# rezashkv/diffusion_pruning

Hardware: AMD Instinct MI355X
Metric: denoise-steps/s (SD-2.1 U-Net forward, 512x512, bs=4 per GPU, 50% channel mask) (higher is better)
Workload: dtype bf16; 1 GPU; BASELINE configs[1]: SD-2.1 UNet2DConditionModelGated.forward, 64x64 latents (512x512), bs=4/GPU, fixed 50% mask (gated semantics), seeded random-init weights, HIP graph replay; global_batch=4, parallelism=replicas x1 (no data-path collective)

## Files before the change

diffusion_pruning_amd/csrc/conv_gemm.hip:

```cpp
#include "conv_gemm_core.h"

using namespace aptp_cg;

namespace {

template <typename T> struct Elem;
template <> struct Elem<__bf16> { static constexpr int EPC = 8, KS = 64; };
template <> struct Elem<float> { static constexpr int EPC = 4, KS = 32; };

template <int BM, int BN, int WM, int WN, typename T = __bf16>
__global__ __launch_bounds__(256) void conv_gemm_kernel(const KParams p) {
  static_assert(WM * WN == 4, "4 waves per workgroup");
  constexpr int EPC = Elem<T>::EPC, KS = Elem<T>::KS, ES = (int)sizeof(T);
  constexpr bool F32 = sizeof(T) == 4;
  constexpr int WTM = BM / WM, WTN = BN / WN;
  constexpr int MF = WTM / 16, NF = WTN / 16;
  constexpr int A_PASS = BM / 32, B_PASS = BN / 32;
  static_assert(BM % 32 == 0 && BN % 32 == 0 && WTM % 16 == 0 && WTN % 16 == 0, "tile shape");

  __shared__ __attribute__((aligned(16))) T smem[2 * (BM + BN) * KS];
  T* As = smem;
  T* Bs = smem + 2 * BM * KS;

  const int tid = threadIdx.x, lane = tid & 63, wave = tid >> 6;
// ... 1016 lines not shown
void launch_tile(const KParams& k, hipStream_t s) {
  const int tiles = ((k.M + BM - 1) / BM) * ((k.N + BN - 1) / BN);
  dim3 grid(tiles * k.split_k, 1, 1);
  if (k.io_f32) hipLaunchKernelGGL((conv_gemm_kernel<BM, BN, 2, 2, float>), grid, dim3(256), 0, s, k);
  else hipLaunchKernelGGL((conv_gemm_kernel<BM, BN, 2, 2>), grid, dim3(256), 0, s, k);
}

template <int BM, int BN, int STAGES>
void launch_tile_dma(const KParams& k, hipStream_t s) {
  const int tiles = ((k.M + BM - 1) / BM) * ((k.N + BN - 1) / BN);
  dim3 grid(tiles * k.split_k, 1, 1);
  hipLaunchKernelGGL((conv_gemm_dma_kernel<BM, BN, 2, 2, STAGES>), grid, dim3(256), 0, s, k);
}

template <int BM, int BN, int WM, int WN, int STAGES = 2>
void launch_tile_dma8(const KParams& k, hipStream_t s) {
  const int tiles = ((k.M + BM - 1) / BM) * ((k.N + BN - 1) / BN);
  dim3 grid(tiles * k.split_k, 1, 1);
  hipLaunchKernelGGL((conv_gemm_dma_kernel<BM, BN, WM, WN, STAGES>), grid, dim3(512), 0, s, k);
}

template <int BM, int BN, int WM, int WN, int STAGES>
void launch_tile_ku2(const KParams& k, hipStream_t s) {
  const int tiles = ((k.M + BM - 1) / BM) * ((k.N + BN - 1) / BN);
  dim3 grid(tiles * k.split_k, 1, 1);
  hipLaunchKernelGGL((conv_gemm_dma_kernel<BM, BN, WM, WN, STAGES, false, 2>), grid, dim3(WM * WN * 64), 0, s, k);
}

template <int BM, int BN, int STAGES>
void launch_tile_ks2(const KParams& k, hipStream_t s) {
  const int tiles = ((k.M + BM - 1) / BM) * ((k.N + BN - 1) / BN);
  dim3 grid(tiles * k.split_k, 1, 1);
  hipLaunchKernelGGL((conv_gemm_dma_kernel<BM, BN, 2, 2, STAGES, false, 1, 2>), grid, dim3(512), 0, s, k);
}

template <int BM, int BN, int WM, int WN, int STAGES>
void launch_tile_pp(const KParams& k, hipStream_t s) {
  const int tiles = ((k.M + BM - 1) / BM) * ((k.N + BN - 1) / BN);
  dim3 grid(tiles * k.split_k, 1, 1);
  hipLaunchKernelGGL((conv_gemm_dma_kernel<BM, BN, WM, WN, STAGES, true>), grid, dim3(512), 0, s, k);
}

}

extern "C" int64_t aptp_conv_gemm_workspace_bytes(const AptpConvGemmParams* p) {
  if (!p || p->split_k <= 1) return 0;
  const int64_t M = (int64_t)p->B * p->Hout * p->Wout;
  const int t = pick_tile(p, (int)M);
  if (is_sk_tile(t))
    return (int64_t)aptp_sk_cus() * 2 * kTiles[t].bm * kTiles[t].bn * (int64_t)sizeof(float);
  int64_t mp = M, np = p->N;
  if (t > 0 && t < kNumTiles) {
    mp = (M + kTiles[t].bm - 1) / kTiles[t].bm * kTiles[t].bm;
    np = ((int64_t)p->N + kTiles[t].bn - 1) / kTiles[t].bn * kTiles[t].bn;
  }
  return (int64_t)p->split_k * mp * np * (int64_t)sizeof(float);
}

extern "C" int aptp_conv_gemm_tiles(const AptpConvGemmParams* p) {
  if (!p) return 0;
  const int64_t M = (int64_t)p->B * p->Hout * p->Wout;
  const int t = pick_tile(p, (int)M);
  if (t <= 0 || t >= kNumTiles) return 0;
  return (int)(((M + kTiles[t].bm - 1) / kTiles[t].bm) * ((p->N + kTiles[t].bn - 1) / kTiles[t].bn));
}

extern "C" int aptp_conv_gemm_colstat_rows(const AptpConvGemmParams* p) {
  if (!p) return 0;
  const int t = pick_tile(p, p->B * p->Hout * p->Wout);
  if (t <= 0 || t >= kNumTiles) return 0;
  return kTiles[t].bm / (kTiles[t].nw / kTiles[t].wn);
}

extern "C" int aptp_conv_gemm_rowstat_slots(const AptpConvGemmParams* p) {
  if (!p) return 0;
  const int t = pick_tile(p, p->B * p->Hout * p->Wout);
  if (t <= 0 || t >= kNumTiles) return 0;
  return ((p->N + kTiles[t].bn - 1) / kTiles[t].bn) * kTiles[t].wn;
}

extern "C" int aptp_conv_gemm_suggest_split_k(const AptpConvGemmParams* p) {
  if (!p) return 1;
  const int M = p->B * p->Hout * p->Wout;
  const int t = pick_tile(p, M);
  const int64_t blocks = (int64_t)((M + kTiles[t].bm - 1) / kTiles[t].bm) * ((p->N + kTiles[t].bn - 1) / kTiles[t].bn);
  const int nK = p->KH * p->KW * (p->cin_pad / BK);
  if (blocks >= 256) return 1;
  int s = (int)((512 + blocks - 1) / blocks);
  const int max_s = nK / 8 > 0 ? nK / 8 : 1;
  if (s > max_s) s = max_s;
  if (s > 32) s = 32;
  return s < 1 ? 1 : s;
}

extern "C" int aptp_conv_gemm(const AptpConvGemmParams* p, aptp_stream_t stream) {
  KParams k;
  const int rc = fill_kparams(p, k);
  if (rc != APTP_OK) return rc;
  if (k.split_k > 1) APTP_CHECK(k.ws != nullptr && ((uintptr_t)k.ws % 16) == 0, "conv_gemm: split_k > 1 needs a 16B-aligned workspace");
  if (k.split_k == 1) k.counters = nullptr;
  k.gn_gamma = p->gn_gamma; k.gn_beta = p->gn_beta; k.gn_groups = p->gn_groups; k.gn_C = p->gn_C; k.gn_silu = p->gn_silu; k.gn_eps = p->gn_eps;
  if (k.gn_gamma) {
    APTP_CHECK(k.gn_beta && k.split_k > 1 && !k.counters && !k.out_f32 && k.act == APTP_ACT_NONE && !k.colgate && !k.corr && !k.residual && !k.depth
               && !k.rstat_out && !k.cstat_out && !k.ln_stats, "conv_gemm: gn_gamma needs a plain bf16 convolution split along K with a reduce launch");
    APTP_CHECK(k.gn_groups > 0 && k.gn_C > 0 && k.gn_C <= k.N && k.gn_C % k.gn_groups == 0 && k.gn_C % 8 == 0 && (k.gn_C / k.gn_groups) % 4 == 0
               && (int64_t)k.HW * (k.gn_C / k.gn_groups) <= 4LL * GN_RED_QPT * GN_RED_NT && k.ldy % 4 == 0,
               "conv_gemm: gn_gamma geometry (C=%d groups=%d HW=%d)", k.gn_C, k.gn_groups, k.HW);
  }
  hipStream_t s = (hipStream_t)stream;
  int t = pick_tile(p, k.M);
  if (t < 0 || t >= kNumTiles) { aptp_set_error("conv_gemm: unknown tile %d", t); return APTP_EINVAL; }
  if (k.io_f32 && t >= APTP_TILE_DMA_128x128) {
    aptp_set_error("conv_gemm: io_f32 (fp32 parity path) runs on the register-staged tiles 1..6 only (got tile %d)", t);
    return APTP_EINVAL;
  }
  if (t >= APTP_TILE_DMA_128x128 && !is_sk_tile(t) && (p->cin_pad * 2 > 8064 || (p->x2 && p->cin2_pad * 2 > 8064))) {
    aptp_set_error("conv_gemm: LDS-DMA tiles need Cin <= 4032 (got cin_pad %d)", p->cin_pad);
    return APTP_EINVAL;
  }
  if (k.rstat_out) {
    const int slots = ((k.N + kTiles[t].bn - 1) / kTiles[t].bn) * kTiles[t].wn;
    if ((k.split_k != 1 && !k.counters) || k.rstat_slots != slots) {
      aptp_set_error("conv_gemm: rowstat_out needs split_k == 1 (or the in-kernel reduction) and rowstat_slots == aptp_conv_gemm_rowstat_slots() (%d), got split_k %d, slots %d",
                     slots, k.split_k, k.rstat_slots);
      return APTP_EINVAL;
    }
  }
  if (k.cstat_out) {
    const int wtm = kTiles[t].bm / (kTiles[t].nw / kTiles[t].wn), wtn = kTiles[t].bn / kTiles[t].wn;
    if (!k.epi16 || k.act == APTP_ACT_GEGLU || (k.split_k != 1 && !k.counters) || k.HW % wtm != 0 || wtn < 32 ||
        k.cstat_ld < k.Nout || ((uintptr_t)k.cstat_out % 8) != 0) {
      aptp_set_error("conv_gemm: colstat_out needs the coalesced bf16 epilogue, no GEGLU, split_k == 1 (or the in-kernel reduction), "
                     "Hout*Wout %% %d == 0 (aptp_conv_gemm_colstat_rows) and colstat_ld >= N", wtm);
      return APTP_EINVAL;
    }
    const int wl = k.act == APTP_ACT_GEGLU ? wtn / 2 : wtn;
    if (k.ustat_out && (wl % k.ustat_unit == 0 ? wl / k.ustat_unit : (wl - 1) / k.ustat_unit + 2) > 64) {
      aptp_set_error("conv_gemm: ustat_unit %d too small for the %d columns of a wave of tile %d (at most 64 units per wave)", k.ustat_unit, wl, t);
      return APTP_EINVAL;
    }
  }
  if (k.act == APTP_ACT_GEGLU && (kTiles[t].bn == 160)) {
    aptp_set_error("conv_gemm: GEGLU cannot use a 160-wide tile");
    return APTP_EINVAL;
  }
  {
    const int tiles_m = (k.M + kTiles[t].bm - 1) / kTiles[t].bm, tiles_n = (k.N + kTiles[t].bn - 1) / kTiles[t].bn;
    APTP_CHECK((int64_t)tiles_m * tiles_n * k.split_k < (1ll << 31) && (int64_t)k.nK * (k.split_k + 1) < (1ll << 31), "conv_gemm: grid too large");
    k.fd_hw = make_fastdiv(k.HW); k.fd_wout = make_fastdiv(k.Wout);
    k.fd_tm = make_fastdiv(tiles_m); k.fd_tn = make_fastdiv(tiles_n); k.fd_sk = make_fastdiv(k.split_k);
    k.fd_perm = make_fastdiv(tiles_n * k.split_k); k.fd_tmn = make_fastdiv(tiles_m * tiles_n);
  }
  static const bool lin_on = !(getenv("APTP_LIN") && getenv("APTP_LIN")[0] == '0');
  if (lin_on && p->epilogue != 2 && p->pad_end == 0 && aptp_lin_eligible(k, t)) {
    const int rc2 = aptp_launch_lin(k, t, s);
    if (rc2 != APTP_OK) return rc2;
    APTP_LAUNCH_CHECK();
    return APTP_OK;
  }
  static const bool lean_on = !(getenv("APTP_CONV_LEAN") && getenv("APTP_CONV_LEAN")[0] == '0');
  if (lean_on && p->epilogue == 0 && p->pad_end == 0 && aptp_conv_lean_eligible(k, t)) {
    const int rc2 = aptp_launch_conv_lean(k, t, s);
    if (rc2 != APTP_OK) return rc2;
  } else
  switch (t) {
    case APTP_TILE_128x128: launch_tile<128, 128>(k, s); break;
    case APTP_TILE_128x160: launch_tile<128, 160>(k, s); break;
    case APTP_TILE_64x128: launch_tile<64, 128>(k, s); break;
    case APTP_TILE_64x160: launch_tile<64, 160>(k, s); break;
    case APTP_TILE_128x64: launch_tile<128, 64>(k, s); break;
    case APTP_TILE_64x64: launch_tile<64, 64>(k, s); break;
    case APTP_TILE_DMA_128x128: launch_tile_dma<128, 128, 2>(k, s); break;
    case APTP_TILE_DMA_128x160: launch_tile_dma<128, 160, 2>(k, s); break;
    case APTP_TILE_DMA_64x128: launch_tile_dma<64, 128, 2>(k, s); break;
    case APTP_TILE_DMA_64x160: launch_tile_dma<64, 160, 2>(k, s); break;
    case APTP_TILE_DMA_128x64: launch_tile_dma<128, 64, 2>(k, s); break;
    case APTP_TILE_DMA_64x64: launch_tile_dma<64, 64, 2>(k, s); break;
    case APTP_TILE_DMA3_128x128: launch_tile_dma<128, 128, 3>(k, s); break;
    case APTP_TILE_DMA3_128x160: launch_tile_dma<128, 160, 3>(k, s); break;
    case APTP_TILE_DMA3_64x128: launch_tile_dma<64, 128, 3>(k, s); break;
    case APTP_TILE_DMA3_64x160: launch_tile_dma<64, 160, 3>(k, s); break;
    case APTP_TILE_DMA3_128x64: launch_tile_dma<128, 64, 3>(k, s); break;
    case APTP_TILE_DMA3_64x64: launch_tile_dma<64, 64, 3>(k, s); break;
    case APTP_TILE_DMA8_128x160: launch_tile_dma8<128, 160, 4, 2>(k, s); break;
    case APTP_TILE_DMA8_256x160: launch_tile_dma8<256, 160, 4, 2>(k, s); break;
    case APTP_TILE_DMA8_128x128: launch_tile_dma8<128, 128, 2, 4>(k, s); break;
    case APTP_TILE_DMA8_256x128: launch_tile_dma8<256, 128, 4, 2>(k, s); break;
    case APTP_TILE_DMA4_64x160: launch_tile_dma<64, 160, 4>(k, s); break;
    case APTP_TILE_DMA4_64x128: launch_tile_dma<64, 128, 4>(k, s); break;
    case APTP_TILE_DMA4_64x64: launch_tile_dma<64, 64, 4>(k, s); break;
    case APTP_TILE_DMA4_128x64: launch_tile_dma<128, 64, 4>(k, s); break;
    case APTP_TILE_DMA4_128x128: launch_tile_dma<128, 128, 4>(k, s); break;
    case APTP_TILE_DMA8R3_128x160: launch_tile_dma8<128, 160, 4, 2, 3>(k, s); break;
    case APTP_TILE_DMA8R4_128x160: launch_tile_dma8<128, 160, 4, 2, 4>(k, s); break;
    case APTP_TILE_DMA8R3_128x128: launch_tile_dma8<128, 128, 2, 4, 3>(k, s); break;
    case APTP_TILE_DMA8R4_128x128: launch_tile_dma8<128, 128, 2, 4, 4>(k, s); break;
    case APTP_TILE_DMA8R3_256x128: launch_tile_dma8<256, 128, 4, 2, 3>(k, s); break;
    case APTP_TILE_PP3_128x160: launch_tile_pp<128, 160, 4, 2, 3>(k, s); break;
    case APTP_TILE_PP4_128x160: launch_tile_pp<128, 160, 4, 2, 4>(k, s); break;
    case APTP_TILE_PP3_128x128: launch_tile_pp<128, 128, 2, 4, 3>(k, s); break;
    case APTP_TILE_PP4_128x128: launch_tile_pp<128, 128, 2, 4, 4>(k, s); break;
    case APTP_TILE_PP4_64x160: launch_tile_pp<64, 160, 4, 2, 4>(k, s); break;
    case APTP_TILE_PP4_64x128: launch_tile_pp<64, 128, 2, 4, 4>(k, s); break;
    case APTP_TILE_PP5_64x160: launch_tile_pp<64, 160, 4, 2, 5>(k, s); break;
    case APTP_TILE_PP4_128x64: launch_tile_pp<128, 64, 4, 2, 4>(k, s); break;
    case APTP_TILE_PP3_256x128: launch_tile_pp<256, 128, 4, 2, 3>(k, s); break;
    case APTP_TILE_PP3_128x256: launch_tile_pp<128, 256, 2, 4, 3>(k, s); break;
    case APTP_TILE_DMA6_64x64: launch_tile_dma<64, 64, 6>(k, s); break;
    case APTP_TILE_DMA8S_64x64: launch_tile_dma<64, 64, 8>(k, s); break;
    case APTP_TILE_DMA6_64x128: launch_tile_dma<64, 128, 6>(k, s); break;
    case APTP_TILE_DMA6_128x64: launch_tile_dma<128, 64, 6>(k, s); break;
    case APTP_TILE_KU2S4_64x64: launch_tile_ku2<64, 64, 2, 2, 4>(k, s); break;
    case APTP_TILE_KU2S6_64x64: launch_tile_ku2<64, 64, 2, 2, 6>(k, s); break;
    case APTP_TILE_KU2S4_64x128: launch_tile_ku2<64, 128, 2, 2, 4>(k, s); break;
    case APTP_TILE_KU2S6_64x128: launch_tile_ku2<64, 128, 2, 2, 6>(k, s); break;
    case APTP_TILE_KU2S4_128x64: launch_tile_ku2<128, 64, 2, 2, 4>(k, s); break;
    case APTP_TILE_KU2S4_128x128: launch_tile_ku2<128, 128, 2, 2, 4>(k, s); break;
    case APTP_TILE_KU2S4_64x160: launch_tile_ku2<64, 160, 2, 2, 4>(k, s); break;
    case APTP_TILE_KU2S4_128x160: launch_tile_ku2<128, 160, 4, 2, 4>(k, s); break;
    case APTP_TILE_KU2S4_128x128W8: launch_tile_ku2<128, 128, 2, 4, 4>(k, s); break;
    case APTP_TILE_KS2S3_64x64: launch_tile_ks2<64, 64, 3>(k, s); break;
    case APTP_TILE_KS2S4_64x64: launch_tile_ks2<64, 64, 4>(k, s); break;
    case APTP_TILE_KS2S3_64x128: launch_tile_ks2<64, 128, 3>(k, s); break;
    case APTP_TILE_KS2S4_64x128: launch_tile_ks2<64, 128, 4>(k, s); break;
    case APTP_TILE_KS2S3_128x64: launch_tile_ks2<128, 64, 3>(k, s); break;
    case APTP_TILE_KS2S3_128x128: launch_tile_ks2<128, 128, 3>(k, s); break;
    case APTP_TILE_SK_256x160: case APTP_TILE_SK_256x128: case APTP_TILE_SK_128x256:
    case APTP_TILE_SKL_256x160: case APTP_TILE_SKL_256x128: case APTP_TILE_SKL_128x256:
    case APTP_TILE_SK_128x160: case APTP_TILE_SKL_128x160: case APTP_TILE_SK_128x128: case APTP_TILE_SKL_128x128: {
      if (k.split_k > 1 && !k.counters) { aptp_set_error("conv_gemm: the stream-K tiles combine in-kernel: split_k > 1 needs tile_counters"); return APTP_EINVAL; }
      const int rc2 = aptp_launch_sk(k, t, s);
      if (rc2 != APTP_OK) return rc2;
      break;
    }
    case APTP_TILE_HALO_128x160:
    case APTP_TILE_HALO_128x128: {
      const int W = p->Wout;
      if (!(p->KH == 3 && p->KW == 3 && p->stride == 1 && p->pad == 1 && p->pad_end == 0 && p->ups == 0 && !p->x2 && W > 0 && 128 % W == 0 &&
            (p->Hout * W) % 128 == 0 && (128 / W + 2) * (W + 2) <= 264)) {
        aptp_set_error("conv_gemm: the halo tiles need a 3x3 / stride-1 / pad-1 convolution without x2 whose width divides 128 (16, 32 or 64)");
        return APTP_EINVAL;
      }
      const int tiles = ((k.M + 127) / 128) * ((k.N + kTiles[t].bn - 1) / kTiles[t].bn);
      if (t == APTP_TILE_HALO_128x160) hipLaunchKernelGGL((conv3x3_halo_kernel<160, 4>), dim3(tiles * k.split_k), dim3(512), 0, s, k);
      else hipLaunchKernelGGL((conv3x3_halo_kernel<128, 4>), dim3(tiles * k.split_k), dim3(512), 0, s, k);
      break;
    }
    default: aptp_set_error("conv_gemm: unknown tile %d", t); return APTP_EINVAL;
  }
  APTP_LAUNCH_CHECK();
  if (k.split_k > 1 && !k.counters) {
    if (k.gn_gamma) {
      hipLaunchKernelGGL(splitk_reduce_gn_kernel, dim3(k.gn_groups, k.B), dim3(GN_RED_NT), 0, s, k);
    } else {
      const int quads = (k.act == APTP_ACT_GEGLU) ? k.N / 8 : k.N / 4;
      const int64_t total = (int64_t)k.M * quads;
      hipLaunchKernelGGL(splitk_reduce_kernel, dim3((unsigned)((total + 255) / 256)), dim3(256), 0, s, k);
    }
    APTP_LAUNCH_CHECK();
  }
  return APTP_OK;
}
```

diffusion_pruning_amd/csrc/lin_gemm.hip:

```cpp
#include "conv_gemm_core.h"

namespace {
using namespace aptp_cg;

__device__ __attribute__((aligned(256))) unsigned char g_lin_zero_page[8192];

typedef __attribute__((address_space(3))) void* lds_ptr;
typedef const __attribute__((address_space(1))) void* gbl_ptr;

template <int BM, int BN, int WM, int WN, int STAGES, int KU, bool GEGLU = false, int GELU = 0>
__global__ __launch_bounds__(WM * WN * 64) void lin_gemm_kernel(const KParams p) {
  constexpr int NW = WM * WN, NT = NW * 64, RPP = NT / 8;
  constexpr int WTM = BM / WM, WTN = BN / WN, MF = WTM / 16, NF = WTN / 16;
  constexpr int A_PASS = BM / RPP, B_PASS = BN / RPP, NLD = A_PASS + B_PASS;
  constexpr int D = STAGES - KU;
  static_assert(BM % RPP == 0 && BN % RPP == 0 && WTM % 16 == 0 && WTN % 32 == 0, "tile shape");
  static_assert(STAGES % KU == 0 && D >= KU && NLD * (D - KU) <= 63, "ring");
  constexpr int WL = GEGLU ? WTN / 2 : WTN;
  constexpr int LPR = WL / 8, RPW = (64 / LPR) < WTM ? (64 / LPR) : WTM, NPASS = WTM / RPW, PITCH = WTN + 4;
  static_assert((LPR & (LPR - 1)) == 0 && WTM % RPW == 0, "transposed layout");
  static_assert(NW * WTM * PITCH * 4 <= STAGES * (BM + BN) * BK * 2, "epilogue transpose buffer");

  __shared__ __attribute__((aligned(16))) __bf16 smem[STAGES * (BM + BN) * BK];
  __shared__ unsigned pf_scratch[64];
  __bf16* As = smem;
  __bf16* Bs = smem + STAGES * BM * BK;

  const int tid = threadIdx.x, lane = tid & 63;
  const int wave = __builtin_amdgcn_readfirstlane(tid >> 6);
  const int wm = wave / WN, wn = wave % WN;
  const int tiles_n = (p.N + BN - 1) / BN, tiles_m = (p.M + BM - 1) / BM;
  int tm, tn;
  {
    const int L = blockIdx.x;
    if (p.order == 0) {
      tm = p.fd_tn.div(L); tn = L - tm * tiles_n;
    } else {
      const int T = gridDim.x, xcd = L & 7, j = L >> 3, qq = T >> 3, r = T & 7;
      const int q = (xcd < r ? xcd * (qq + 1) : r * (qq + 1) + (xcd - r) * qq) + j;
      if (p.order == 1) { tn = p.fd_tm.div(q); tm = q - tn * tiles_m; }
      else { tm = p.fd_tn.div(q); tn = q - tm * tiles_n; }
    }
  }
  const int m0 = tm * BM, n0 = tn * BN;
  const int nk = p.ncc;

  const int rowbase = tid >> 3;
  const int schunk = (tid & 7) ^ ((rowbase >> 1) & 7);
  const char* const zpage = reinterpret_cast<const char*>(g_lin_zero_page) + schunk * 16;
  const bool tail_bad = ((nk - 1) * BK + schunk * 8) >= p.Cin;
  const char* a_ptr[A_PASS];
  const char* b_ptr[B_PASS];
#pragma unroll
  for (int i = 0; i < A_PASS; ++i) {
    const int m = m0 + rowbase + RPP * i;
    const char* va = reinterpret_cast<const char*>(p.x) + ((int64_t)m * p.ldx + schunk * 8) * 2;
    a_ptr[i] = m < p.M ? va : zpage;
  }
#pragma unroll
  for (int i = 0; i < B_PASS; ++i) {
    int n = n0 + rowbase + RPP * i;
    n = n < p.N ? n : p.N - 1;
    b_ptr[i] = reinterpret_cast<const char*>(p.w) + ((int64_t)n * p.Ktot + schunk * 8) * 2;
  }
  auto issue_tile = [&](int t, int stage) {
    const bool pad = (t == nk - 1) && tail_bad;
#pragma unroll
    for (int i = 0; i < A_PASS; ++i) {
      const char* src = pad ? zpage : a_ptr[i];
      __bf16* dst = As + (stage * BM + wave * 8 + RPP * i) * BK;
      __builtin_amdgcn_global_load_lds((gbl_ptr)src, (lds_ptr)dst, 16, 0, 0);
      a_ptr[i] += BK * 2;
    }
#pragma unroll
    for (int i = 0; i < B_PASS; ++i) {
      __bf16* dst = Bs + (stage * BN + wave * 8 + RPP * i) * BK;
      __builtin_amdgcn_global_load_lds((gbl_ptr)b_ptr[i], (lds_ptr)dst, 16, 0, 0);
      b_ptr[i] += BK * 2;
    }
  };
  if (p.pf_ptr) {
    const int xcd = blockIdx.x & 7;
    const int x0 = (int)(((int64_t)p.pf_lines * xcd) >> 3), x1 = (int)(((int64_t)p.pf_lines * (xcd + 1)) >> 3);
    const int l0 = x0 + (int)(blockIdx.x >> 3) * p.pf_per;
    const int l1 = l0 + p.pf_per < x1 ? l0 + p.pf_per : x1;
    for (int l = l0 + tid; l < l1; l += NT)
      __builtin_amdgcn_global_load_lds((gbl_ptr)(p.pf_ptr + (int64_t)l * 64), (lds_ptr)pf_scratch, 4, 0, 0);
  }

  const int pre = nk < D ? nk : D;
#pragma unroll
  for (int t = 0; t < D; ++t)
    if (t < pre) issue_tile(t, t);

  const int lrow = lane / LPR, lc8 = lane - lrow * LPR;
  const int c0 = (GEGLU ? ((n0 + wn * WTN) >> 1) : (n0 + wn * WTN)) + lc8 * 8;
  const bool col_on = c0 < p.Nout && lrow < RPW;
  const int c0c = c0 < p.Nout ? c0 : p.Nout - 8;
  const int pc = GEGLU ? ((c0c >> 4) * 32 + (c0c & 15)) : c0c;
  const int bofs = GEGLU ? ((lc8 >> 1) * 32 + (lc8 & 1) * 8) : lc8 * 8;
  int mrow[NPASS];
  u32x4 rres[NPASS];
#pragma unroll
  for (int ps = 0; ps < NPASS; ++ps) {
    const int m2 = m0 + wm * WTM + ps * RPW + lrow;
    mrow[ps] = m2 < p.M ? m2 : p.M - 1;
    rres[ps] = (u32x4){0u, 0u, 0u, 0u};
  }
  if (p.residual) {
#pragma unroll
    for (int ps = 0; ps < NPASS; ++ps) rres[ps] = *reinterpret_cast<const u32x4*>(p.residual + (int64_t)mrow[ps] * p.ldres + c0c);
  }
  float4 bia[2] = {make_float4(0.f, 0.f, 0.f, 0.f), make_float4(0.f, 0.f, 0.f, 0.f)};
  float4 csm[2] = {make_float4(0.f, 0.f, 0.f, 0.f), make_float4(0.f, 0.f, 0.f, 0.f)};
  float4 biag[2] = {make_float4(0.f, 0.f, 0.f, 0.f), make_float4(0.f, 0.f, 0.f, 0.f)};
  float4 csmg[2] = {make_float4(0.f, 0.f, 0.f, 0.f), make_float4(0.f, 0.f, 0.f, 0.f)};
  if (p.bias) {
    bia[0] = *reinterpret_cast<const float4*>(p.bias + pc);
    bia[1] = *reinterpret_cast<const float4*>(p.bias + pc + 4);
    if constexpr (GEGLU) {
      biag[0] = *reinterpret_cast<const float4*>(p.bias + pc + 16);
      biag[1] = *reinterpret_cast<const float4*>(p.bias + pc + 20);
    }
  }
  float ln_mean[NPASS], ln_rstd[NPASS];
#pragma unroll
  for (int ps = 0; ps < NPASS; ++ps) { ln_mean[ps] = 0.f; ln_rstd[ps] = 1.f; }
  if (p.ln_stats) {
    csm[0] = *reinterpret_cast<const float4*>(p.ln_colsum + pc);
    csm[1] = *reinterpret_cast<const float4*>(p.ln_colsum + pc + 4);
    if constexpr (GEGLU) {
      csmg[0] = *reinterpret_cast<const float4*>(p.ln_colsum + pc + 16);
      csmg[1] = *reinterpret_cast<const float4*>(p.ln_colsum + pc + 20);
    }
    const float4* sp = reinterpret_cast<const float4*>(p.ln_stats);
    const int npair = p.ln_slots >> 1;
    float a[NPASS], a2[NPASS];
#pragma unroll
    for (int ps = 0; ps < NPASS; ++ps) { a[ps] = 0.f; a2[ps] = 0.f; }
    constexpr int UNR = 3;
    for (int base = 0; base < npair; base += UNR * LPR) {
      float4 t[UNR][NPASS];
#pragma unroll
      for (int u = 0; u < UNR; ++u) {
        if (base + u * LPR < npair) {
          const int pr = base + u * LPR + lc8;
          const int64_t row0 = (int64_t)(pr < npair ? pr : 0) * p.M;
#pragma unroll
          for (int ps = 0; ps < NPASS; ++ps) t[u][ps] = sp[row0 + mrow[ps]];
        } else {
#pragma unroll
          for (int ps = 0; ps < NPASS; ++ps) t[u][ps] = make_float4(0.f, 0.f, 0.f, 0.f);
        }
      }
#pragma unroll
      for (int u = 0; u < UNR; ++u) {
        const bool ok = base + u * LPR + lc8 < npair;
#pragma unroll
        for (int ps = 0; ps < NPASS; ++ps) {
          a[ps] += ok ? t[u][ps].x + t[u][ps].z : 0.f;
          a2[ps] += ok ? t[u][ps].y + t[u][ps].w : 0.f;
        }
      }
    }
#pragma unroll
    for (int ps = 0; ps < NPASS; ++ps) {
#pragma unroll
      for (int off = 1; off < LPR; off <<= 1) { a[ps] += __shfl_xor(a[ps], off); a2[ps] += __shfl_xor(a2[ps], off); }
      const float mean = a[ps] * p.ln_invC;
      float var = a2[ps] * p.ln_invC - mean * mean;
      var = var < 0.f ? 0.f : var;
      ln_mean[ps] = mean;
      ln_rstd[ps] = rsqrtf(var + p.ln_eps);
    }
  }
  f32x4 acc[MF][NF];
#pragma unroll
  for (int i = 0; i < MF; ++i)
#pragma unroll
    for (int j = 0; j < NF; ++j) acc[i][j] = (f32x4){0.f, 0.f, 0.f, 0.f};
  const int frow = lane & 15, fq = lane >> 4;
  auto compute = [&](int stage) {
#pragma unroll
    for (int s = 0; s < 2; ++s) {
      bf16x8 af[MF], wf[NF];
#pragma unroll
      for (int i = 0; i < MF; ++i) {
        const int r = wm * WTM + i * 16 + frow;
        af[i] = *reinterpret_cast<const bf16x8*>(As + (stage * BM + r) * BK + ((s * 4 + fq) ^ ((r >> 1) & 7)) * 8);
      }
#pragma unroll
      for (int j = 0; j < NF; ++j) {
        const int r = wn * WTN + j * 16 + frow;
        wf[j] = *reinterpret_cast<const bf16x8*>(Bs + (stage * BN + r) * BK + ((s * 4 + fq) ^ ((r >> 1) & 7)) * 8);
      }
#pragma unroll
      for (int i = 0; i < MF; ++i)
#pragma unroll
        for (int j = 0; j < NF; ++j) acc[i][j] = __builtin_amdgcn_mfma_f32_16x16x32_bf16(wf[j], af[i], acc[i][j], 0, 0, 0);
    }
  };

  if (pre == D && D > KU) asm volatile("s_waitcnt vmcnt(%0)" ::"n"(NLD * (D - KU)) : "memory");
  else asm volatile("s_waitcnt vmcnt(0)" ::: "memory");
  __builtin_amdgcn_s_barrier();
  asm volatile("" ::: "memory");
  {
    int cur = 0, nxt = D;
    const int nfull = nk / KU;
    for (int it = 0; it < nfull; ++it) {
      const int kt = it * KU;
#pragma unroll
      for (int u = 0; u < KU; ++u)
        if (kt + D + u < nk) issue_tile(kt + D + u, nxt + u);
      compute(cur);
      if constexpr (KU == 2) compute(cur + 1);
      asm volatile("" ::: "memory");
      if (kt + D + KU <= nk && D > KU) asm volatile("s_waitcnt vmcnt(%0)" ::"n"(NLD * (D - KU)) : "memory");
      else asm volatile("s_waitcnt vmcnt(0)" ::: "memory");
      asm volatile("s_waitcnt lgkmcnt(0)" ::: "memory");
      __builtin_amdgcn_s_barrier();
      asm volatile("" ::: "memory");
      cur = cur + KU == STAGES ? 0 : cur + KU;
      nxt = nxt + KU == STAGES ? 0 : nxt + KU;
    }
    if constexpr (KU == 2) {
      if (nk & 1) {
        compute(cur);
        asm volatile("s_waitcnt lgkmcnt(0)" ::: "memory");
        __builtin_amdgcn_s_barrier();
        asm volatile("" ::: "memory");
      }
    }
  }

  float* const buf = reinterpret_cast<float*>(smem) + wave * (WTM * PITCH);
#pragma unroll
  for (int i = 0; i < MF; ++i)
#pragma unroll
    for (int j = 0; j < NF; ++j)
      *reinterpret_cast<f32x4*>(buf + (i * 16 + frow) * PITCH + j * 16 + fq * 4) = acc[i][j];
  __builtin_amdgcn_fence(__ATOMIC_ACQ_REL, "wavefront");
  __builtin_amdgcn_wave_barrier();
  __bf16* const yb = reinterpret_cast<__bf16*>(p.y);
  float cs[8], cs2[8];
#pragma unroll
  for (int e = 0; e < 8; ++e) { cs[e] = 0.f; cs2[e] = 0.f; }
  const int slot = tn * WN + wn;
#pragma unroll
  for (int ps = 0; ps < NPASS; ++ps) {
    const int r = (ps * RPW + lrow) < WTM ? (ps * RPW + lrow) : 0, m2 = m0 + wm * WTM + r;
    const bool on = col_on && m2 < p.M;
    float v[8], gt[8];
    {
      const float4 a = *reinterpret_cast<const float4*>(buf + r * PITCH + bofs);
      const float4 b = *reinterpret_cast<const float4*>(buf + r * PITCH + bofs + 4);
      v[0] = a.x; v[1] = a.y; v[2] = a.z; v[3] = a.w; v[4] = b.x; v[5] = b.y; v[6] = b.z; v[7] = b.w;
    }
    if constexpr (GEGLU) {
      const float4 a = *reinterpret_cast<const float4*>(buf + r * PITCH + bofs + 16);
      const float4 b = *reinterpret_cast<const float4*>(buf + r * PITCH + bofs + 20);
      gt[0] = a.x; gt[1] = a.y; gt[2] = a.z; gt[3] = a.w; gt[4] = b.x; gt[5] = b.y; gt[6] = b.z; gt[7] = b.w;
    }
    const float cb[8] = {bia[0].x, bia[0].y, bia[0].z, bia[0].w, bia[1].x, bia[1].y, bia[1].z, bia[1].w};
    if (p.ln_stats) {
      const float cc[8] = {csm[0].x, csm[0].y, csm[0].z, csm[0].w, csm[1].x, csm[1].y, csm[1].z, csm[1].w};
#pragma unroll
      for (int e = 0; e < 8; ++e) v[e] = ln_rstd[ps] * (v[e] - ln_mean[ps] * cc[e]);
      if constexpr (GEGLU) {
        const float cg[8] = {csmg[0].x, csmg[0].y, csmg[0].z, csmg[0].w, csmg[1].x, csmg[1].y, csmg[1].z, csmg[1].w};
#pragma unroll
        for (int e = 0; e < 8; ++e) gt[e] = ln_rstd[ps] * (gt[e] - ln_mean[ps] * cg[e]);
      }
    }
#pragma unroll
    for (int e = 0; e < 8; ++e) v[e] += cb[e];
    if constexpr (GEGLU) {
      const float cbg[8] = {biag[0].x, biag[0].y, biag[0].z, biag[0].w, biag[1].x, biag[1].y, biag[1].z, biag[1].w};
#pragma unroll
      for (int e = 0; e < 8; ++e) v[e] = v[e] * gelu_erf_f(gt[e] + cbg[e]);
    } else
    if constexpr (GELU == 1) {
#pragma unroll
      for (int e = 0; e < 8; ++e) v[e] = gelu_erf_f(v[e]);
    } else
    if constexpr (GELU == 2) {
#pragma unroll
      for (int e = 0; e < 8; ++e) v[e] = quick_gelu_f(v[e]);
    } else
    if (p.act == APTP_ACT_SILU) {
#pragma unroll
      for (int e = 0; e < 8; ++e) v[e] = silu_f(v[e]);
    }
    if (p.residual) {
      float f[8];
      union { u32x4 v; uint4 s; } cv; cv.v = rres[ps];
      unpack_bf16x8(cv.s, f);
#pragma unroll
      for (int e = 0; e < 8; ++e) v[e] += f[e];
    }
    const uint4 o = pack_bf16x8(v);
    if (on) *reinterpret_cast<uint4*>(yb + (int64_t)m2 * p.ldy + c0) = o;
    if (p.cstat_out || p.rstat_out) {
      float f[8];
      unpack_bf16x8(o, f);
      if (p.cstat_out && on) {
#pragma unroll
        for (int e = 0; e < 8; ++e) { cs[e] += f[e]; cs2[e] += f[e] * f[e]; }
      }
      if (p.rstat_out) {
        float s0 = 0.f, s1 = 0.f;
        if (col_on) {
#pragma unroll
          for (int e = 0; e < 8; ++e) { s0 += f[e]; s1 += f[e] * f[e]; }
        }
#pragma unroll
        for (int off = 1; off < LPR; off <<= 1) { s0 += __shfl_xor(s0, off); s1 += __shfl_xor(s1, off); }
        if (m2 < p.M && lc8 == 0) {
          float2 q; q.x = s0; q.y = s1;
          reinterpret_cast<float2*>(p.rstat_out)[((int64_t)(slot >> 1) * p.M + m2) * 2 + (slot & 1)] = q;
        }
      }
    }
  }
  if (!GEGLU && p.cstat_out) {
    static_assert(RPW * WTN <= WTM * PITCH, "column-statistics staging");
    float tot[2][(WTN + 63) / 64];
#pragma unroll
    for (int ph = 0; ph < 2; ++ph) {
      __builtin_amdgcn_fence(__ATOMIC_ACQ_REL, "wavefront");
      __builtin_amdgcn_wave_barrier();
      float* dst = buf + lrow * WTN + lc8 * 8;
      if (ph == 0) {
        *reinterpret_cast<float4*>(dst) = make_float4(cs[0], cs[1], cs[2], cs[3]);
        *reinterpret_cast<float4*>(dst + 4) = make_float4(cs[4], cs[5], cs[6], cs[7]);
      } else {
        *reinterpret_cast<float4*>(dst) = make_float4(cs2[0], cs2[1], cs2[2], cs2[3]);
        *reinterpret_cast<float4*>(dst + 4) = make_float4(cs2[4], cs2[5], cs2[6], cs2[7]);
      }
      __builtin_amdgcn_fence(__ATOMIC_ACQ_REL, "wavefront");
      __builtin_amdgcn_wave_barrier();
#pragma unroll
      for (int q = 0; q < (WTN + 63) / 64; ++q) {
        const int t = lane + 64 * q;
        float a = 0.f;
        if (t < WTN) {
#pragma unroll
          for (int r = 0; r < RPW; ++r) a += buf[r * WTN + t];
        }
        tot[ph][q] = a;
      }
    }
    const int cw0 = n0 + wn * WTN;
    float2* dstg = reinterpret_cast<float2*>(p.cstat_out) + (int64_t)(m0 / WTM + wm) * p.cstat_ld;
#pragma unroll
    for (int q = 0; q < (WTN + 63) / 64; ++q) {
      const int t = lane + 64 * q;
      if (t < WTN && cw0 + t < p.Nout) dstg[cw0 + t] = make_float2(tot[0][q], tot[1][q]);
    }
    if constexpr (!GEGLU) {
      if (p.ustat_out) emit_unit_stats<WTN>(p, tot, buf, lane, cw0, m0 + wm * WTM);
    }
  }
}

template <int BM, int BN, int WM, int WN, int STAGES, int KU>
void launch_lin(KParams k, hipStream_t s) {
  const bool geglu = k.act == APTP_ACT_GEGLU;
  const int tiles = ((k.M + BM - 1) / BM) * ((k.N + BN - 1) / BN);
  k.pf_lines = 0; k.pf_per = 0;
  if (k.pf_ptr) {
    const int nper = (tiles + 7) >> 3;
    k.pf_lines = (int)(k.pf_bytes >> 6);
    const int per_xcd = (k.pf_lines + 7) >> 3;
    k.pf_per = (per_xcd + nper - 1) / nper;
    if (k.pf_per < 1) k.pf_per = 1;
  }
  if (geglu) hipLaunchKernelGGL((lin_gemm_kernel<BM, BN, WM, WN, STAGES, KU, true>), dim3(tiles), dim3(WM * WN * 64), 0, s, k);
  else if (k.act == APTP_ACT_GELU) hipLaunchKernelGGL((lin_gemm_kernel<BM, BN, WM, WN, STAGES, KU, false, 1>), dim3(tiles), dim3(WM * WN * 64), 0, s, k);
  else if (k.act == APTP_ACT_QUICK_GELU) hipLaunchKernelGGL((lin_gemm_kernel<BM, BN, WM, WN, STAGES, KU, false, 2>), dim3(tiles), dim3(WM * WN * 64), 0, s, k);
  else hipLaunchKernelGGL((lin_gemm_kernel<BM, BN, WM, WN, STAGES, KU, false>), dim3(tiles), dim3(WM * WN * 64), 0, s, k);
}

}

namespace aptp_cg {

bool aptp_lin_eligible(const KParams& k, int tile) {
  if (k.KH != 1 || k.KW != 1 || k.stride != 1 || k.pad != 0 || k.ups != 0 || k.zins || k.x2 || k.ncc2) return false;
  if (k.split_k != 1 || k.io_f32 || k.out_f32 || !k.epi16 || k.gn_gamma) return false;
  if (k.colgate || k.corr || k.rowbias || k.depth) return false;
  if (k.act == APTP_ACT_GEGLU && (k.residual || k.rstat_out || k.cstat_out || k.N % 32 != 0)) return false;
  if (k.Nout < 8 || k.ncc < 1) return false;
  switch (tile) {
    case APTP_TILE_DMA_64x64: case APTP_TILE_DMA3_64x64: case APTP_TILE_DMA4_64x64: case APTP_TILE_DMA6_64x64: case APTP_TILE_DMA8S_64x64:
    case APTP_TILE_KU2S4_64x64: case APTP_TILE_KU2S6_64x64:
    case APTP_TILE_DMA_64x128: case APTP_TILE_DMA3_64x128: case APTP_TILE_DMA4_64x128: case APTP_TILE_DMA6_64x128:
    case APTP_TILE_KU2S4_64x128: case APTP_TILE_KU2S6_64x128:
    case APTP_TILE_DMA_128x64: case APTP_TILE_DMA3_128x64: case APTP_TILE_DMA4_128x64: case APTP_TILE_DMA6_128x64: case APTP_TILE_KU2S4_128x64:
      return true;
    default: return false;
  }
}

int aptp_launch_lin(const KParams& k, int tile, hipStream_t s) {
  switch (tile) {
    case APTP_TILE_DMA_64x64: launch_lin<64, 64, 2, 2, 2, 1>(k, s); break;
    case APTP_TILE_DMA3_64x64: launch_lin<64, 64, 2, 2, 3, 1>(k, s); break;
    case APTP_TILE_DMA4_64x64: case APTP_TILE_DMA6_64x64: case APTP_TILE_DMA8S_64x64: launch_lin<64, 64, 2, 2, 4, 1>(k, s); break;
    case APTP_TILE_KU2S4_64x64: case APTP_TILE_KU2S6_64x64: launch_lin<64, 64, 2, 2, 4, 2>(k, s); break;
    case APTP_TILE_DMA_64x128: launch_lin<64, 128, 2, 2, 2, 1>(k, s); break;
    case APTP_TILE_DMA3_64x128: launch_lin<64, 128, 2, 2, 3, 1>(k, s); break;
    case APTP_TILE_DMA4_64x128: case APTP_TILE_DMA6_64x128: launch_lin<64, 128, 2, 2, 4, 1>(k, s); break;
    case APTP_TILE_KU2S4_64x128: case APTP_TILE_KU2S6_64x128: launch_lin<64, 128, 2, 2, 4, 2>(k, s); break;
    case APTP_TILE_DMA_128x64: launch_lin<128, 64, 2, 2, 2, 1>(k, s); break;
    case APTP_TILE_DMA3_128x64: launch_lin<128, 64, 2, 2, 3, 1>(k, s); break;
    case APTP_TILE_DMA4_128x64: case APTP_TILE_DMA6_128x64: launch_lin<128, 64, 2, 2, 4, 1>(k, s); break;
    case APTP_TILE_KU2S4_128x64: launch_lin<128, 64, 2, 2, 4, 2>(k, s); break;
    default: aptp_set_error("lin_gemm: tile %d has no lean instantiation", tile); return APTP_EINVAL;
  }
  return APTP_OK;
}

}
```

diffusion_pruning_amd/launch_policy.py:

```python
import json
import math
import os
import re

from . import _lib as L

BK = 64
DMA_TILE_FIRST = L.TILE_DMA_128x128
DMA_MAX_CHANNELS = 4032
SK_TILE_FIRST = L.TILE_SK_256x160
SK_MAX_CHANNELS = 32704
_HALO_TILES = (L.TILE_HALO_128x160, L.TILE_HALO_128x128)
_LEAN_TILES = frozenset(getattr(L, "TILE_" + t) for t in (
    "DMA_64x128 DMA_128x64 DMA_64x64 DMA3_64x128 DMA3_128x64 DMA3_64x64 DMA4_64x128 DMA4_64x64 DMA4_128x64 DMA6_64x64 DMA8S_64x64 "
    "DMA6_64x128 DMA6_128x64 KU2S4_64x64 KU2S6_64x64 KU2S4_64x128 KU2S6_64x128 KU2S4_128x64").split())

TUNING_NEAREST = os.environ.get("APTP_TUNING_NEAREST", "1") != "0"
TUNING_MAX_DIST = 2.0
LEAN_REMAP = os.environ.get("APTP_LEAN_REMAP", "1") != "0"
SK_AUTO = os.environ.get("APTP_SK_AUTO", "1") == "1"
SK_AUTO_MIN_OUTPUTS = 256 * 256 * 160
SK_AUTO_MIN_KSTEPS = 16
SPLITK_FORCE_IN_KERNEL = os.environ.get("APTP_SPLITK_FORCE_INKERNEL", "0") == "1"
COLS_SPLIT_MAX = int(os.environ.get("APTP_COLS_SPLIT_MAX", "2"))

_KEY = re.compile(r"M(\d+)_N(\d+)_C(\d+)_T(\d+)_s(\d+)u(\d+)g(\d+)(?:x(\d+))?$")


def tuning_key(M, N, Cin, taps, stride, ups, geglu, Cin2: int = 0) -> str:
    return f"M{M}_N{N}_C{Cin}_T{taps}_s{stride}u{ups}g{int(bool(geglu))}" + (f"x{Cin2}" if Cin2 else "")


def parse_key(key: str):
    m = _KEY.match(key)
    return m and tuple(int(t) if t else 0 for t in m.groups())


def key_of(p) -> str:
    return tuning_key(p.B * p.Hout * p.Wout, p.N, p.Cin, p.KH * p.KW, p.stride, p.ups, p.act == L.ACT_GEGLU, p.Cin2 if p.x2 else 0)


_path = os.environ.get("APTP_TUNING") or os.path.join(os.path.dirname(os.path.abspath(__file__)), "tuning_gfx950.json")
TUNING = {}
if os.path.exists(_path):
    with open(_path) as _f:
        TUNING.update(json.load(_f))
_classes = None
_near = {}


def invalidate():
    global _classes
    _classes = None
    _near.clear()


def set_tuning(table):
    table = dict(table)
    TUNING.clear()
    TUNING.update(table)
    invalidate()


def set_entry(key: str, entry):
    if entry is None:
        TUNING.pop(key, None)
    else:
        TUNING[key] = entry
    invalidate()


def _nearest(key, M, N, Cin, taps, stride, ups, geglu, Cin2):
    global _classes
    if key in _near:
        return _near[key]
    if _classes is None:
        _classes = {}
        for k, v in TUNING.items():
            s = parse_key(k)
            if s is not None:
                _classes.setdefault((s[3], s[4], s[5], s[6], s[7] > 0), []).append((s[0], s[1], s[3] * s[2] + s[7], v))
    K = taps * Cin + Cin2
    best, bd = None, TUNING_MAX_DIST
    for (M2, N2, K2, v) in _classes.get((taps, stride, ups, int(bool(geglu)), Cin2 > 0), ()):
        if v["tile"] in _HALO_TILES and M2 != M:
            continue
        if v["tile"] >= DMA_TILE_FIRST and max(Cin, Cin2) > DMA_MAX_CHANNELS:
            continue
        dm = math.log2(M / M2)
        d = (0.5 * dm if dm > 0 else -1.5 * dm) + abs(math.log2(N / N2)) + abs(math.log2(K / K2))
        if d < bd:
            best, bd = v, d
    if best is not None:
        nK = (K + BK - 1) // BK
        best = dict(best)
        best["split_k"] = max(1, min(int(best["split_k"]), nK // 4 if nK >= 8 else 1))
    _near[key] = best
    return best


def tuning_lookup(M, N, Cin, taps, stride, ups, geglu, Cin2: int = 0):
    key = tuning_key(M, N, Cin, taps, stride, ups, geglu, Cin2)
    hit = TUNING.get(key)
    if hit is None and TUNING_NEAREST:
        hit = _nearest(key, M, N, Cin, taps, stride, ups, geglu, Cin2)
    return hit


def _lean_tile(M):
    return L.TILE_DMA_128x64 if M >= 8192 else (L.TILE_DMA3_64x64 if M >= 2048 else L.TILE_KU2S4_64x64)


def choose_launch(M, N, Cin, cin_pad, KH, KW, stride, ups, act, Cin2, cin2_pad, *, plain_linear, f32, tile, split_k, order):
    if split_k is not None or tile != 0 or f32:
        return tile, split_k, None, order
    taps, geglu = KH * KW, act == L.ACT_GEGLU
    channels = max(cin_pad, cin2_pad)
    sk_sized = SK_AUTO and M * N >= SK_AUTO_MIN_OUTPUTS and taps * (cin_pad // BK) + cin2_pad // BK >= SK_AUTO_MIN_KSTEPS
    lean = LEAN_REMAP and plain_linear and cin_pad <= DMA_MAX_CHANNELS
    key = tuning_key(M, N, Cin, taps, stride, ups, geglu, Cin2)
    tuned = TUNING.get(key)
    if tuned is None and TUNING_NEAREST:
        tuned = _nearest(key, M, N, Cin, taps, stride, ups, geglu, Cin2)
        if tuned is not None and sk_sized:
            tuned = None
    if tuned is not None and tuned["tile"] >= DMA_TILE_FIRST \
            and channels > (SK_MAX_CHANNELS if tuned["tile"] >= SK_TILE_FIRST else DMA_MAX_CHANNELS):
        tuned = None
    if tuned is not None:
        tile = tuned["tile"]
        if lean and tile not in _LEAN_TILES and tuned["split_k"] == 1 and "insitu" not in tuned:
            tile = _lean_tile(M)
        return tile, tuned["split_k"], bool(tuned.get("in_kernel", 0)), order or tuned.get("order", 1)
    if lean and not (M <= 512 and cin_pad >= 1280):
        return _lean_tile(M), 1, None, order
    if sk_sized and channels <= SK_MAX_CHANNELS:
        return (L.TILE_SK_256x128 if geglu else L.TILE_SK_256x160), 2, True, order or 3
    return 0, None, None, order


def splitk_in_kernel(split_k, in_kernel, *, explicit, reduce_launch, rowstats, colstats) -> bool:
    if reduce_launch:
        return False
    if SPLITK_FORCE_IN_KERNEL:
        return True
    if in_kernel is None:
        in_kernel = split_k <= 4 or explicit
    return in_kernel or rowstats or (colstats and split_k <= COLS_SPLIT_MAX)
```

Before: 207.1 steps/s.

## Add split-K support to the linear GEMM kernel with in-kernel combine

Adds a SPLIT template variant of lin_gemm_kernel. It decodes a k-slice per block, offsets the A and B pointers to that K range, and reduces partial sums through splitk_combine before running the epilogue. Epilogue operand loads (residual, bias, LN stats) are deferred until after the combine in split mode, so blocks that are not the final reducer skip them. The eligibility check now allows split_k>1 when a workspace and counters exist, and the launch policy keeps tuned split-K entries on lean tiles unless APTP_LIN_SPLITK=0. The goal is more parallelism for small-M, large-K linears, at the cost of workspace traffic and cross-block synchronization.

```diff
diff --git a/diffusion_pruning_amd/csrc/conv_gemm.hip b/diffusion_pruning_amd/csrc/conv_gemm.hip
--- a/diffusion_pruning_amd/csrc/conv_gemm.hip
+++ b/diffusion_pruning_amd/csrc/conv_gemm.hip
@@ -1192,7 +1192,7 @@
     k.fd_perm = make_fastdiv(tiles_n * k.split_k); k.fd_tmn = make_fastdiv(tiles_m * tiles_n);
   }
   static const bool lin_on = !(getenv("APTP_LIN") && getenv("APTP_LIN")[0] == '0');
-  if (lin_on && p->epilogue != 2 && p->pad_end == 0 && aptp_lin_eligible(k, t)) {
+  if (lin_on && p->epilogue != 2 && p->pad_end == 0 && p->split_k <= k.nK && aptp_lin_eligible(k, t)) {
     const int rc2 = aptp_launch_lin(k, t, s);
     if (rc2 != APTP_OK) return rc2;
     APTP_LAUNCH_CHECK();
diff --git a/diffusion_pruning_amd/csrc/lin_gemm.hip b/diffusion_pruning_amd/csrc/lin_gemm.hip
--- a/diffusion_pruning_amd/csrc/lin_gemm.hip
+++ b/diffusion_pruning_amd/csrc/lin_gemm.hip
@@ -8,7 +8,7 @@
 typedef __attribute__((address_space(3))) void* lds_ptr;
 typedef const __attribute__((address_space(1))) void* gbl_ptr;
 
-template <int BM, int BN, int WM, int WN, int STAGES, int KU, bool GEGLU = false, int GELU = 0>
+template <int BM, int BN, int WM, int WN, int STAGES, int KU, bool GEGLU = false, int GELU = 0, bool SPLIT = false>
 __global__ __launch_bounds__(WM * WN * 64) void lin_gemm_kernel(const KParams p) {
   constexpr int NW = WM * WN, NT = NW * 64, RPP = NT / 8;
   constexpr int WTM = BM / WM, WTN = BN / WN, MF = WTM / 16, NF = WTN / 16;
@@ -30,8 +30,10 @@
   const int wave = __builtin_amdgcn_readfirstlane(tid >> 6);
   const int wm = wave / WN, wn = wave % WN;
   const int tiles_n = (p.N + BN - 1) / BN, tiles_m = (p.M + BM - 1) / BM;
-  int tm, tn;
-  {
+  int tm, tn, kz = 0;
+  if constexpr (SPLIT) {
+    decode_block(p, tiles_m, tiles_n, tm, tn, kz);
+  } else {
     const int L = blockIdx.x;
     if (p.order == 0) {
       tm = p.fd_tn.div(L); tn = L - tm * tiles_n;
@@ -43,28 +45,32 @@
     }
   }
   const int m0 = tm * BM, n0 = tn * BN;
-  const int nk = p.ncc;
+  int kb = 0, nk = p.ncc;
+  if constexpr (SPLIT) {
+    kb = p.fd_sk.div(p.nK * kz);
+    nk = p.fd_sk.div(p.nK * (kz + 1)) - kb;
+  }
 
   const int rowbase = tid >> 3;
   const int schunk = (tid & 7) ^ ((rowbase >> 1) & 7);
   const char* const zpage = reinterpret_cast<const char*>(g_lin_zero_page) + schunk * 16;
-  const bool tail_bad = ((nk - 1) * BK + schunk * 8) >= p.Cin;
+  const bool tail_bad = ((p.ncc - 1) * BK + schunk * 8) >= p.Cin;
   const char* a_ptr[A_PASS];
   const char* b_ptr[B_PASS];
 #pragma unroll
   for (int i = 0; i < A_PASS; ++i) {
     const int m = m0 + rowbase + RPP * i;
     const char* va = reinterpret_cast<const char*>(p.x) + ((int64_t)m * p.ldx + schunk * 8) * 2;
-    a_ptr[i] = m < p.M ? va : zpage;
+    a_ptr[i] = (m < p.M ? va : zpage) + kb * (BK * 2);
   }
 #pragma unroll
   for (int i = 0; i < B_PASS; ++i) {
     int n = n0 + rowbase + RPP * i;
     n = n < p.N ? n : p.N - 1;
-    b_ptr[i] = reinterpret_cast<const char*>(p.w) + ((int64_t)n * p.Ktot + schunk * 8) * 2;
+    b_ptr[i] = reinterpret_cast<const char*>(p.w) + ((int64_t)n * p.Ktot + kb * BK + schunk * 8) * 2;
   }
   auto issue_tile = [&](int t, int stage) {
-    const bool pad = (t == nk - 1) && tail_bad;
+    const bool pad = (kb + t == p.ncc - 1) && tail_bad;
 #pragma unroll
     for (int i = 0; i < A_PASS; ++i) {
       const char* src = pad ? zpage : a_ptr[i];
@@ -107,14 +113,18 @@
     mrow[ps] = m2 < p.M ? m2 : p.M - 1;
     rres[ps] = (u32x4){0u, 0u, 0u, 0u};
   }
-  if (p.residual) {
-#pragma unroll
-    for (int ps = 0; ps < NPASS; ++ps) rres[ps] = *reinterpret_cast<const u32x4*>(p.residual + (int64_t)mrow[ps] * p.ldres + c0c);
-  }
   float4 bia[2] = {make_float4(0.f, 0.f, 0.f, 0.f), make_float4(0.f, 0.f, 0.f, 0.f)};
   float4 csm[2] = {make_float4(0.f, 0.f, 0.f, 0.f), make_float4(0.f, 0.f, 0.f, 0.f)};
   float4 biag[2] = {make_float4(0.f, 0.f, 0.f, 0.f), make_float4(0.f, 0.f, 0.f, 0.f)};
   float4 csmg[2] = {make_float4(0.f, 0.f, 0.f, 0.f), make_float4(0.f, 0.f, 0.f, 0.f)};
+  float ln_mean[NPASS], ln_rstd[NPASS];
+#pragma unroll
+  for (int ps = 0; ps < NPASS; ++ps) { ln_mean[ps] = 0.f; ln_rstd[ps] = 1.f; }
+  auto request_epi = [&]() {
+  if (p.residual) {
+#pragma unroll
+    for (int ps = 0; ps < NPASS; ++ps) rres[ps] = *reinterpret_cast<const u32x4*>(p.residual + (int64_t)mrow[ps] * p.ldres + c0c);
+  }
   if (p.bias) {
     bia[0] = *reinterpret_cast<const float4*>(p.bias + pc);
     bia[1] = *reinterpret_cast<const float4*>(p.bias + pc + 4);
@@ -123,9 +133,6 @@
       biag[1] = *reinterpret_cast<const float4*>(p.bias + pc + 20);
     }
   }
-  float ln_mean[NPASS], ln_rstd[NPASS];
-#pragma unroll
-  for (int ps = 0; ps < NPASS; ++ps) { ln_mean[ps] = 0.f; ln_rstd[ps] = 1.f; }
   if (p.ln_stats) {
     csm[0] = *reinterpret_cast<const float4*>(p.ln_colsum + pc);
     csm[1] = *reinterpret_cast<const float4*>(p.ln_colsum + pc + 4);
@@ -174,6 +181,13 @@
       ln_rstd[ps] = rsqrtf(var + p.ln_eps);
     }
   }
+  };
+  #ifdef LIN_SPLIT_EPI_EARLY
+  constexpr bool epi_early = true;
+#else
+  constexpr bool epi_early = !SPLIT;
+#endif
+  if constexpr (epi_early) request_epi();
   f32x4 acc[MF][NF];
 #pragma unroll
   for (int i = 0; i < MF; ++i)
@@ -234,6 +248,10 @@
     }
   }
 
+  if constexpr (SPLIT) {
+    if (!splitk_combine<NT, MF, NF>(p, acc, tm * tiles_n + tn, kz, tid, reinterpret_cast<int*>(smem))) return;
+    if constexpr (!epi_early) request_epi();
+  }
   float* const buf = reinterpret_cast<float*>(smem) + wave * (WTM * PITCH);
 #pragma unroll
   for (int i = 0; i < MF; ++i)
@@ -367,7 +385,7 @@
 template <int BM, int BN, int WM, int WN, int STAGES, int KU>
 void launch_lin(KParams k, hipStream_t s) {
   const bool geglu = k.act == APTP_ACT_GEGLU;
-  const int tiles = ((k.M + BM - 1) / BM) * ((k.N + BN - 1) / BN);
+  const int tiles = ((k.M + BM - 1) / BM) * ((k.N + BN - 1) / BN) * k.split_k;
   k.pf_lines = 0; k.pf_per = 0;
   if (k.pf_ptr) {
     const int nper = (tiles + 7) >> 3;
@@ -376,10 +394,18 @@
     k.pf_per = (per_xcd + nper - 1) / nper;
     if (k.pf_per < 1) k.pf_per = 1;
   }
-  if (geglu) hipLaunchKernelGGL((lin_gemm_kernel<BM, BN, WM, WN, STAGES, KU, true>), dim3(tiles), dim3(WM * WN * 64), 0, s, k);
-  else if (k.act == APTP_ACT_GELU) hipLaunchKernelGGL((lin_gemm_kernel<BM, BN, WM, WN, STAGES, KU, false, 1>), dim3(tiles), dim3(WM * WN * 64), 0, s, k);
-  else if (k.act == APTP_ACT_QUICK_GELU) hipLaunchKernelGGL((lin_gemm_kernel<BM, BN, WM, WN, STAGES, KU, false, 2>), dim3(tiles), dim3(WM * WN * 64), 0, s, k);
-  else hipLaunchKernelGGL((lin_gemm_kernel<BM, BN, WM, WN, STAGES, KU, false>), dim3(tiles), dim3(WM * WN * 64), 0, s, k);
+  const dim3 grid(tiles), block(WM * WN * 64);
+  if (k.split_k > 1) {
+    if (geglu) hipLaunchKernelGGL((lin_gemm_kernel<BM, BN, WM, WN, STAGES, KU, true, 0, true>), grid, block, 0, s, k);
+    else if (k.act == APTP_ACT_GELU) hipLaunchKernelGGL((lin_gemm_kernel<BM, BN, WM, WN, STAGES, KU, false, 1, true>), grid, block, 0, s, k);
+    else if (k.act == APTP_ACT_QUICK_GELU) hipLaunchKernelGGL((lin_gemm_kernel<BM, BN, WM, WN, STAGES, KU, false, 2, true>), grid, block, 0, s, k);
+    else hipLaunchKernelGGL((lin_gemm_kernel<BM, BN, WM, WN, STAGES, KU, false, 0, true>), grid, block, 0, s, k);
+    return;
+  }
+  if (geglu) hipLaunchKernelGGL((lin_gemm_kernel<BM, BN, WM, WN, STAGES, KU, true>), grid, block, 0, s, k);
+  else if (k.act == APTP_ACT_GELU) hipLaunchKernelGGL((lin_gemm_kernel<BM, BN, WM, WN, STAGES, KU, false, 1>), grid, block, 0, s, k);
+  else if (k.act == APTP_ACT_QUICK_GELU) hipLaunchKernelGGL((lin_gemm_kernel<BM, BN, WM, WN, STAGES, KU, false, 2>), grid, block, 0, s, k);
+  else hipLaunchKernelGGL((lin_gemm_kernel<BM, BN, WM, WN, STAGES, KU, false>), grid, block, 0, s, k);
 }
 
 }
@@ -388,7 +414,8 @@
 
 bool aptp_lin_eligible(const KParams& k, int tile) {
   if (k.KH != 1 || k.KW != 1 || k.stride != 1 || k.pad != 0 || k.ups != 0 || k.zins || k.x2 || k.ncc2) return false;
-  if (k.split_k != 1 || k.io_f32 || k.out_f32 || !k.epi16 || k.gn_gamma) return false;
+  if (k.io_f32 || k.out_f32 || !k.epi16 || k.gn_gamma) return false;
+  if (k.split_k != 1 && (k.split_k < 1 || !k.ws || !k.counters || k.split_k > k.ncc)) return false;
   if (k.colgate || k.corr || k.rowbias || k.depth) return false;
   if (k.act == APTP_ACT_GEGLU && (k.residual || k.rstat_out || k.cstat_out || k.N % 32 != 0)) return false;
   if (k.Nout < 8 || k.ncc < 1) return false;
diff --git a/diffusion_pruning_amd/launch_policy.py b/diffusion_pruning_amd/launch_policy.py
--- a/diffusion_pruning_amd/launch_policy.py
+++ b/diffusion_pruning_amd/launch_policy.py
@@ -18,6 +18,7 @@
 TUNING_NEAREST = os.environ.get("APTP_TUNING_NEAREST", "1") != "0"
 TUNING_MAX_DIST = 2.0
 LEAN_REMAP = os.environ.get("APTP_LEAN_REMAP", "1") != "0"
+LIN_SPLITK = os.environ.get("APTP_LIN_SPLITK", "1") != "0"
 SK_AUTO = os.environ.get("APTP_SK_AUTO", "1") == "1"
 SK_AUTO_MIN_OUTPUTS = 256 * 256 * 160
 SK_AUTO_MIN_KSTEPS = 16
@@ -131,7 +132,11 @@
         tile = tuned["tile"]
         if lean and tile not in _LEAN_TILES and tuned["split_k"] == 1 and "insitu" not in tuned:
             tile = _lean_tile(M)
-        return tile, tuned["split_k"], bool(tuned.get("in_kernel", 0)), order or tuned.get("order", 1)
+        split, in_kernel, tord = tuned["split_k"], bool(tuned.get("in_kernel", 0)), tuned.get("order", 1)
+        if plain_linear and tile in _LEAN_TILES and split > 1 and not LIN_SPLITK:
+            was = tuned.get("unsplit", {})
+            tile, split, in_kernel, tord = was.get("tile", tile), 1, False, was.get("order", tord)
+        return tile, split, in_kernel, order or tord
     if lean and not (M <= 512 and cin_pad >= 1280):
         return _lean_tile(M), 1, None, order
     if sk_sized and channels <= SK_MAX_CHANNELS:
```

Result: slower. 203.6 steps/s (-1.7%).
